# wwood/CoverM

Measured on AMD Instinct MI355X. Metric: aligned reads/s through coverm contig (mean trimmed_mean covered_fraction variance), higher is better.
Workload: dtype i32 depth / u64 sums / f32 estimators

## Files before the change

### coverm_amd/csrc/covermhip.hip

```cpp
#include "pileup_kernels.hip.h"
#include "prep_lean.hip.h"
#include "genome_kernels.hip.h"
#include "sep_kernels.hip.h"
#include "ingest_kernels.hip.h"
#include "group_kernels.hip.h"
#include "sam_kernels.hip.h"
#include "gene_kernels.hip.h"
#include "depth_kernels.hip.h"
#include "depth_bins_kernels.hip.h"
#include "depth_regions_kernels.hip.h"

#include <algorithm>
#include <atomic>
#include <cstddef>
#include <chrono>
#include <cstdio>
#include <dlfcn.h>
#include <functional>
#include <sched.h>
#include <cstdlib>
#include <cstring>
#include <map>
#include <mutex>
#include <string>
// ... 1152 lines not shown
    time_begin(s, COV_K_PREP);
    s->last_gen_all = p.gen_all;
    launch_prep_key((p.want_id ? 4 : 0) | (s->cfg.filter_single ? 2 : 0) | (v.mask != nullptr ? 1 : 0), s, p, v);
    if (v.nT) {
        const u32 n_red = p.gen_all ? 0u : (v.nT + 3u) / 4u, cx_grid0 = (u32)s->n_cus * 8u;
        hipLaunchKernelGGL(k_post_prep, dim3(n_red + cx_grid0), dim3(256), 0, v.st, v.r, s->d_tlen.p, s->d_glob.p, v.cx, v.ti, s->d_ctg.p, v.nT, (const PrepPartial *)s->d_part.p,
                           p.prep_grid, p.prep_chunk, n_red);
    }
    time_end(s, COV_K_PREP);
    HIPCHK(hipGetLastError());
    return COV_OK;
}

static cov_status stage_identity_side(cov_session *s, const PassViews &v) {
    const u32 R = v.R, nT = v.nT;
    if (!s->side) {
        (void)ingest_prep_wait(s);
        if (s->ing.aux && !s->ing.active) s->side = s->ing.aux;
        else { HIPCHK(hipStreamCreateWithFlags(&s->side, hipStreamNonBlocking)); s->side_owned = true; }
    }
    HIPCHK(hipEventRecord(s->ev_prep_done, v.st));
    HIPCHK(hipStreamWaitEvent(s->side, s->ev_prep_done, 0));
    (void)hipEventRecord(s->ev[COV_K_IDENTITY][0], s->side);
    if (s->id_mode) {
        const u32 nch = (R + ID_CH - 1) / ID_CH;
        hipLaunchKernelGGL(k_id_approx, dim3(nch), dim3(256), 0, s->side, v.idp, v.idn, R, s->d_idch.p);
        hipLaunchKernelGGL(k_id_predict, dim3(nT), dim3(64), 0, s->side, s->d_ctg.p, nT, v.idp, v.idn, s->d_idch.p);
        hipLaunchKernelGGL(k_id_exact, dim3(nch), dim3(256), 0, s->side, v.idp, v.idn, R, s->d_idch.p);
        hipLaunchKernelGGL(k_id_combine, dim3(nT), dim3(64), 0, s->side, s->d_ctg.p, nT, v.idp, v.idn, v.r.tid, s->d_idch.p);
    } else
        hipLaunchKernelGGL(k_identity, dim3(nT), dim3(64), 0, s->side, s->d_ctg.p, nT, v.idp, v.idn, v.r.tid);
    (void)hipEventRecord(s->ev[COV_K_IDENTITY][1], s->side);
    s->k_launches[COV_K_IDENTITY]++;
    HIPCHK(hipGetLastError());
    HIPCHK(hipEventRecord(s->ev_side_done, s->side));
    s->ev_fresh = -1;
    return COV_OK;
}

static cov_status stage_ranges(cov_session *s, const FinishPlan &p, const PassViews &v) {
    time_begin(s, COV_K_RANGES);
    const u32 n_blocks = (s->n_tiles + 1023u) / 1024u;
    const u32 cx_grid = (u32)s->n_cus * 8u;
    ScanPair sp{};
    sp.cnt[0] = s->d_tcnt.p; sp.scan[0] = s->d_tscan.p; sp.top[0] = s->d_ttop.p; sp.total[0] = nullptr;
    sp.cnt[1] = s->d_cx_cnt.p; sp.scan[1] = s->d_cx_scan.p; sp.top[1] = s->d_cx_top.p; sp.total[1] = &s->d_glob.p->cx_total;
    hipLaunchKernelGGL(k_tile_scan1, dim3(2u * n_blocks), dim3(1024), 0, v.st, sp, s->n_tiles, n_blocks);
    hipLaunchKernelGGL(k_tile_scan2, dim3(2), dim3(1024), 0, v.st, sp, n_blocks);
    hipLaunchKernelGGL((k_cx_expand<true>), dim3(cx_grid), dim3(256), 0, v.st, v.r, s->d_tlen.p, s->d_glob.p, v.cx, v.ti);
    u32 *slow_list = s->use_fast ? s->d_slow_list.p : nullptr;
    u32 *deep_list = const_cast<u32 *>(pileup_deep_list(s));
    const auto ranges = p.want_hist ? &k_ranges<true> : &k_ranges<false>;
    hipLaunchKernelGGL(ranges, dim3((s->n_tiles + 255) / 256), dim3(256), 0, v.st, s->d_tile_contig.p, s->d_tile_start.p, s->n_tiles, s->d_tlen.p,
                       v.mask, s->d_ctg.p, s->d_desc.p, v.ti, s->d_tscan.p, s->d_ttop.p, v.cx, s->d_glob.p, slow_list, deep_list, s->deep_min);
    time_end(s, COV_K_RANGES);
    HIPCHK(hipGetLastError());
    return COV_OK;
}

static cov_status stage_hist_layout(cov_session *s, const PassViews &v) {
    time_begin(s, COV_K_HIST);
    const u32 hb = (v.nT + 1023u) / 1024u;
    HIPCHK(s->d_hist_top.reserve(hb, v.st));
    hipLaunchKernelGGL((k_hist_sum<0>), dim3(hb), dim3(1024), 0, v.st, (const DevContig *)s->d_ctg.p, v.nT, s->d_tlen.p, v.mask, v.excl, s->d_hist_top.p);
    hipLaunchKernelGGL((k_hist_off<0>), dim3(hb), dim3(1024), 0, v.st, s->d_ctg.p, v.nT, s->d_tlen.p, v.mask, v.excl, (const u64 *)s->d_hist_top.p, s->d_glob.p);
    hipLaunchKernelGGL(k_zero_u32, dim3(2048), dim3(256), 0, v.st, s->d_arena.p, &s->d_glob.p->hist_cap_total);
    time_end(s, COV_K_HIST);
    HIPCHK(hipGetLastError());
    return COV_OK;
}

static cov_status stage_pileup(cov_session *s, const FinishPlan &p, const PassViews &v) {
    const PileupArgs a = pileup_args(s);
    time_begin(s, COV_K_PILEUP);
    if (p.want_hist) launch_any_pileup<true, false>(s, a, s->n_tiles);
    else launch_any_pileup<false, false>(s, a, s->n_tiles);
    if (p.hist_stats_launch) {
        const auto hist_stats = p.est_lanes ? &k_hist_stats<true> : &k_hist_stats<false>;
        hipLaunchKernelGGL(hist_stats, dim3(p.est_lanes ? (v.nT + 255) / 256 : (v.nT + 3) / 4), dim3(256), 0, v.st, s->d_ctg.p, v.nT, (const u32 *)s->d_tlen.p,
                           v.mask, v.excl, (const u32 *)s->d_arena.p);
    }
    time_end(s, COV_K_PILEUP);
    HIPCHK(hipGetLastError());
    return COV_OK;
}

static cov_status stage_hist_compact(cov_session *s, const FinishPlan &p, const PassViews &v) {
    s->hist_prefetched = 0;
    if (p.compacted) {
        HIPCHK(s->d_chist.reserve((size_t)v.R + v.nT + 1, v.st));
        time_begin(s, COV_K_HIST_COMPACT);
        launch_hist_compact(s, v.mask, v.excl);
        time_end(s, COV_K_HIST_COMPACT);
        HIPCHK(hipGetLastError());
        const u64 guess = p.hist_prefetch ? std::min<u64>({s->last_chist_total + s->last_chist_total / 16, (u64)v.R + v.nT + 1, (u64)(64u << 20) / 8}) : 0;
        if (guess) {
            if (guess > s->h_chist_cap) HIPCHK(pinned_grow(s->h_chist, s->h_chist_cap, guess));
            HIPCHK(hipMemcpyAsync(s->h_chist, s->d_chist.p, (size_t)guess * 8, hipMemcpyDeviceToHost, v.st));
            s->hist_prefetched = guess;
        }
    }
    s->hist_fetch_seen = false;
    return COV_OK;
}

static cov_status result_host_bind(cov_session *s, const FinishPlan &p, const PassViews &v) {
    result_host_take(s);
// ... 2110 lines not shown
```

### coverm_amd/csrc/pileup_kernels.hip.h

```cpp
#pragma once
#include <hip/hip_runtime.h>
#include <stdint.h>

#define HSTC_FN __host__ __device__ __forceinline__
#include "hist_stats_core.h"
#define PSCHED_FN __host__ __device__ __forceinline__
#include "pileup_schedule_core.h"
#include "scan_ops.hip.h"

namespace covk {

typedef unsigned long long u64;
typedef unsigned int u32;

constexpr u32 F_POS_UNSORTED = 1u;
constexpr u32 RW_SINGLE = 0u, RW_DOUBLE = 1u, RW_COMPLEX = 2u, RW_BUCKET = 3u;
constexpr u32 FAST_MAX_CAND = 8191u;
constexpr u32 TILE_F_GENERIC = 1u, TILE_F_SLOW = 2u, TILE_F_DEEP = 4u;
constexpr u32 CX_MIN_OPS = 16;

struct DevContig {
    u64 n_primary, n_pass, n_nonsupp, sum_nm, sum_indel;
    double id_primary, id_nonsupp;
    u64 sum_d, sum_d2, cov_win, cov_full, proc_win;
    u64 hist_off;
    u32 first_rec, last_rec;
    u32 rec_start, rec_end;
    u32 n_groups;
    u32 max_span;
    u32 flags;
    u32 hist_cap;
    u32 min_d, max_d;
    u32 hist_len;
    u32 cov_out;
    u64 chist_off;
};
static_assert(sizeof(DevContig) == 160, "DevContig layout");

constexpr u32 COUNTER_SLOTS = 64;
struct DevGlobal {
    u64 first_error;
    u64 hist_cap_total;
    u64 chist_total;
    u32 internal_error;
    u32 n_cx;
    u64 cx_total;
    u32 n_slow;
    u32 n_gen;
    u64 pad2[2];
    u64 prim_slots[COUNTER_SLOTS * 8];
    u64 cons_slots[COUNTER_SLOTS * 8];
    u32 n_deep;
    u32 pad_q[8 * 16 - 1];
};

struct FilterCfg {
    u32 include_improper_pairs, include_supplementary, include_secondary;
    u32 filter_single, min_mapq, min_aligned_length;
    float min_percent_identity, min_aligned_percent;
};

struct Records {
    const int32_t *tid, *pos;
    const uint16_t *flag;
    const uint8_t *mapq;
    const u32 *nm;
    const uint8_t *nm_kind;
    const u32 *l_seq;
    const u32 *cigar_off;
    const u32 *cigar;
    u32 n;
// ... 621 lines not shown
        const u32 L = tlen[tid], t0 = ti.tile_first[tid];
        long long cur0 = r.pos[i];
        u32 wd_next = (u32)lane < nops ? r.cigar[co0 + (u32)lane] : 4u;
        for (u32 base = 0; base < nops; base += 64) {
            const u32 wd = wd_next;
            const u32 idn = base + 64u + (u32)lane;
            wd_next = idn < nops ? r.cigar[co0 + idn] : 4u;
            const u32 len = wd >> 4, bit = 1u << (wd & 15u);
            const u32 fr = (bit & 0x18du) ? len : 0u;
            const u32 incl = (u32)wave_incl_scan((int)fr), excl = incl - fr;
            const long long sj = cur0 + (long long)excl;
            const bool m = (bit & 0x181u) != 0u && len > 0u && sj >= 0 && sj < (long long)L;
            const u32 sv = (u32)sj, ev = sv + len;
            const u32 ts = sv >> ti.shift, te = m ? (min(ev, L) - 1u) >> ti.shift : 0u;
            for (u32 k = 0; __any(m && ts + k <= te); k++) {
                const bool v = m && ts + k <= te;
                const u32 key = t0 + ts + k;
                u32 slot = 0;
                for (u64 todo = __ballot(v); todo != 0;) {
                    const int l = __ffsll((long long)todo) - 1;
                    const u32 k0 = __builtin_amdgcn_readlane(key, l);
                    const u64 grp = __ballot(v && key == k0);
                    u32 b = 0;
                    if (lane == l) b = atomicAdd(FILL ? &cx.cur[k0] : &cx.cnt[k0], (u32)__popcll(grp));
                    if (FILL) {
                        b = __builtin_amdgcn_readlane(b, l);
                        if (v && key == k0) slot = b + (u32)__popcll(grp & lt);
                    }
                    todo &= ~grp;
                }
                if (FILL && v) cx.runs[(u64)cx.cscan[key] + cx.ctop[key >> 10] + slot] = make_uint2(sv, ev);
            }
            cur0 += (long long)__builtin_amdgcn_readlane(incl, 63);
        }
    }
}

template <bool FILL>
__global__ __launch_bounds__(256) void k_cx_expand(Records r, const u32 *__restrict__ tlen, DevGlobal *g, CxIdx cx, TileIdx ti) {
    cx_expand_body<FILL>(r, tlen, g, cx, ti, blockIdx.x * 4u + (threadIdx.x >> 6), gridDim.x * 4u);
}

__global__ __launch_bounds__(256) void k_post_prep(Records r, const u32 *__restrict__ tlen, DevGlobal *g, CxIdx cx, TileIdx ti, DevContig *ctg, u32 n_targets,
                                                   const PrepPartial *__restrict__ part, u32 n_parts, u32 chunk_recs, u32 n_red) {
    if (blockIdx.x < n_red) prep_reduce_body(blockIdx.x * 4u + (threadIdx.x >> 6), ctg, n_targets, part, n_parts, chunk_recs);
    else cx_expand_body<false>(r, tlen, g, cx, ti, (blockIdx.x - n_red) * 4u + (threadIdx.x >> 6), (gridDim.x - n_red) * 4u);
}

template <bool WANT_HIST>
__global__ __launch_bounds__(256) void k_ranges(const u32 *__restrict__ tile_contig, const u32 *__restrict__ tile_start,
                                                u32 n_tiles, const u32 *__restrict__ tlen, const uint8_t *__restrict__ mask,
                                                DevContig *ctg, uint4 *__restrict__ desc, TileIdx ti,
                                                const u32 *__restrict__ tscan, const u32 *__restrict__ ttop, CxIdx cx,
                                                DevGlobal *__restrict__ g, u32 *__restrict__ slow_list, u32 *__restrict__ deep_list, u32 deep_min) {
    const u32 t = blockIdx.x * blockDim.x + threadIdx.x;
    if (t >= n_tiles) return;
    const u32 c = tile_contig[t];
    DevContig *C = &ctg[c];
    uint4 out = make_uint4(0u, 0u, tlen[c], 0u);
    u32 cxn = 0, cxo = 0;
    if (C->n_pass != 0 && (mask == nullptr || mask[c])) {
        const u32 rs = C->rec_start, re = C->rec_end;
        cxn = g->cx_total <= cx.runs_cap ? cx.cnt[t] : 0u;
        cxo = cx.cscan[t] + cx.ctop[t >> 10];
        if (C->n_groups != 1u) out.w = 1u;
        if (C->n_groups != 1u || (C->flags & F_POS_UNSORTED)) {
            out.x = rs; out.y = re;
        } else {
            const u32 tf = ti.tile_first[c];
            const u32 before = (tscan[t] + ttop[t >> 10]) - (tscan[tf] + ttop[tf >> 10]);
            const u32 f = rs + before;
            out.y = min(f + ti.tcnt[t], re);
            out.x = max(min(f, ti.fov[t]), rs);
            out.x = min(out.x, out.y);
        }
    }
    if (out.x < out.y || cxn) {
        if (out.w || out.y - out.x + cxn > FAST_MAX_CAND) {
            out.w |= TILE_F_SLOW;
            if (slow_list != nullptr) slow_list[atomicAdd(&g->n_slow, 1u)] = t;
        }
    }
    if (deep_list != nullptr) {
        const bool deep = (out.x < out.y || cxn) && !(out.w & TILE_F_SLOW) && out.y - out.x + cxn >= deep_min;
        const u64 dm = __ballot(deep);
        if (dm != 0ull) {
            const int lane = lane_id(), lead = __ffsll((long long)dm) - 1;
            u32 base = 0;
            if (lane == lead) base = atomicAdd(&g->n_deep, (u32)__popcll(dm));
            base = (u32)__builtin_amdgcn_readlane((int)base, lead);
            if (deep) {
                out.w |= TILE_F_DEEP;
                deep_list[base + (u32)__popcll(dm & (lane == 0 ? 0ull : (~0ull >> (64 - lane))))] = t;
            }
        }
    }
    if (WANT_HIST) {
        const u32 npass = (u32)min(C->n_pass, (u64)0xffffffffu);
        const u32 cap = min(out.y - out.x + cxn, npass);
        if (__all(c == (u32)__builtin_amdgcn_readfirstlane((int)c))) {
            const u32 m = wave_max_u32(cap);
            if (lane_id() == 0 && m) atomicMax(&C->hist_cap, m);
        } else if (cap) atomicMax(&C->hist_cap, cap);
    }
    desc[2 * t] = out;
    desc[2 * t + 1] = make_uint4(c, tile_start[t], cxo, cxn);
}

template <int MODE>
__device__ __forceinline__ u64 hist_bins_of(const DevContig *C, u32 c, const u32 *__restrict__ tlen, const uint8_t *__restrict__ mask, u64 excl) {
    const bool live = C->n_pass != 0 && (mask == nullptr || mask[c]);
    if (MODE == 0) return live ? (u64)C->hist_cap + 1 : 0;
    return (live && 2 * excl < (u64)tlen[c]) ? (u64)C->max_d + 1 : 0;
}
template <int MODE>
__global__ __launch_bounds__(1024) void k_hist_sum(const DevContig *__restrict__ ctg, u32 n_targets, const u32 *__restrict__ tlen,
                                                   const uint8_t *__restrict__ mask, u64 excl, u64 *__restrict__ top) {
    __shared__ u64 wtot[16];
    const u32 c = blockIdx.x * 1024u + threadIdx.x;
    u64 total;
    (void)block_incl_scan<16>(c < n_targets ? hist_bins_of<MODE>(&ctg[c], c, tlen, mask, excl) : 0ull, wtot, total);
    if (threadIdx.x == 0) top[blockIdx.x] = total;
}
template <int MODE>
__global__ __launch_bounds__(1024) void k_hist_off(DevContig *ctg, u32 n_targets, const u32 *__restrict__ tlen, const uint8_t *__restrict__ mask,
                                                   u64 excl, const u64 *__restrict__ top, DevGlobal *g) {
    __shared__ u64 wtot[16];
    const u64 base = blocks_in_front<16>(top, wtot);
    const u32 c = blockIdx.x * 1024u + threadIdx.x;
    const u64 v = c < n_targets ? hist_bins_of<MODE>(&ctg[c], c, tlen, mask, excl) : 0;
    u64 total;
    const u64 inc = block_incl_scan<16>(v, wtot, total);
    if (c < n_targets) {
        if (MODE == 0) ctg[c].hist_off = base + inc - v;
        else { ctg[c].chist_off = base + inc - v; ctg[c].hist_len = (u32)v; }
    }
    if (blockIdx.x == gridDim.x - 1 && threadIdx.x == 0) {
        if (MODE == 0) g->hist_cap_total = base + total; else g->chist_total = base + total;
    }
}

__global__ void k_zero_u32(u32 *__restrict__ p, const u64 *__restrict__ n_ptr) {
    const u64 n = *n_ptr;
    for (u64 i = (u64)blockIdx.x * blockDim.x + threadIdx.x; i < n; i += (u64)gridDim.x * blockDim.x) p[i] = 0u;
}

__global__ __launch_bounds__(256) void k_hist_compact(const DevContig *__restrict__ ctg, u32 n_targets,
                                                      const u32 *__restrict__ tlen, u64 excl,
                                                      const u32 *__restrict__ arena, u64 *__restrict__ out) {
    const u32 c = blockIdx.x * 4u + (threadIdx.x >> 6);
    if (c >= n_targets) return;
    const DevContig *C = &ctg[c];
    const u32 n = C->hist_len;
    if (n == 0) return;
    const u64 win_len = (u64)tlen[c] - 2 * excl;
    for (u32 d = threadIdx.x & 63u; d < n; d += 64u) {
        u64 v = arena[C->hist_off + d];
        if (d == 0) v += win_len - C->proc_win;
        out[C->chist_off + d] = v;
// ... 521 lines not shown

template <bool WANT_HIST, int HB, int TABLES>
__device__ __forceinline__ void pileup_fast_body(const PileupArgs &a, u32 n_tiles, u32 chunk_tiles, const u32 *__restrict__ deep_list, const u32 *__restrict__ n_deep_ptr) {
    constexpr int TW = FAST_TW, HBW = HB;
    constexpr int DS = TABLES == 1 ? 2 : 0;
    constexpr size_t WB = (size_t)TW * 2 * TABLES + (WANT_HIST ? (size_t)HBW * 4 : 0);
    extern __shared__ __attribute__((aligned(16))) char smem[];
    const int lane = threadIdx.x & 63, w = threadIdx.x >> 6;
    u32 *S = reinterpret_cast<u32 *>(smem + (size_t)w * WB);
    u32 *E = TABLES == 2 ? S + TW / 2 : S;
    u32 *lhist = S + (TW / 2) * TABLES;
    uint4 *S4 = reinterpret_cast<uint4 *>(S), *E4 = reinterpret_cast<uint4 *>(E);
    const u32 wpb = blockDim.x >> 6;
    const u32 wave_id = (u32)__builtin_amdgcn_readfirstlane((int)(blockIdx.x * wpb + (u32)w)), n_waves = gridDim.x * wpb;
    if (WANT_HIST) {
#pragma unroll
        for (int b = lane; b < HBW; b += 64) lhist[b] = 0u;
    }
    u64 sum_d = 0, sum_d2 = 0, proc_win = 0;
    u32 cov_w = 0, cov_f = 0, mn = 0xffffffffu, mx = 0;
    u32 cov_o = 0;
    int cur_c = -1;
    u64 hoff = 0; u32 hcap = 0;
    const u64 excl = a.excl;
    u32 hbound = 0;
    auto drain = [&]() {
        lds_fence();
        for (u32 b = (u32)lane; b <= hbound; b += 64) {
            const u32 x = lhist[b];
            if (x) { atomicAdd(&a.hist_arena[hoff + b], x); lhist[b] = 0u; }
        }
        lds_fence();
        hbound = 0;
    };

    auto hist_add = [&](u32 d, u32 x) {
        if (__builtin_expect(d < (u32)HBW, 1)) atomicAdd(&lhist[d], x);
        else hist_add_overflow(a.hist_arena, hoff, hcap, a.g, d, x);
    };
    auto flush = [&]() {
        if (WANT_HIST) {
            if (cur_c >= 0) {
                drain();
                if (__any(cov_o != 0u)) {
                    const u32 co = wave_sum_u32_dpp(cov_o);
                    if (lane == 0) atomicAdd(&a.ctg[cur_c].cov_out, co);
                }
            }
            cov_o = 0; hbound = 0;
            return;
        }
        if (cur_c >= 0) {
            const bool narrow = !__any((sum_d | sum_d2) >> 50);
            const u64 s1 = narrow ? wave_sum_u56(sum_d) : wave_sum_u64(sum_d), s2 = narrow ? wave_sum_u56(sum_d2) : wave_sum_u64(sum_d2);
            const u32 c1 = wave_sum_u32_dpp(cov_w), c2 = wave_sum_u32_dpp(cov_f);
            const u32 m1 = wave_min_u32_dpp(mn), m2 = wave_max_u32_dpp(mx);
            DevContig *C = &a.ctg[cur_c];
            if (lane == 0) {
                if (s1) atomicAdd(&C->sum_d, s1);
                if (s2) atomicAdd(&C->sum_d2, s2);
                if (c1) atomicAdd(&C->cov_win, (u64)c1);
                if (c2) atomicAdd(&C->cov_full, (u64)c2);
                if (proc_win) {
                    atomicAdd(&C->proc_win, proc_win);
                    atomicMin(&C->min_d, m1);
                    atomicMax(&C->max_d, m2);
                }
            }
        }
        sum_d = sum_d2 = 0; proc_win = 0; cov_w = cov_f = 0; mn = 0xffffffffu; mx = 0;
    };
    auto load_runs = [&](const uint4 &d, uint2 &r0, uint2 &r1) {
        const u32 i0 = d.x + (u32)lane, i1 = i0 + 64u;
        r0 = i0 < d.y ? a.runs[i0] : make_uint2(0u, 0u);
        r1 = i1 < d.y ? a.runs[i1] : make_uint2(0u, 0u);
    };
    const psched::Launch sched = psched::launch_of(n_tiles, chunk_tiles, n_waves, deep_list != nullptr ? *n_deep_ptr : 0u);
    const u32 skip_flags = TILE_F_SLOW | (deep_list != nullptr ? TILE_F_DEEP : 0u);
    psched::Visit vis = psched::first(sched, wave_id);
    if (vis.done) return;
    u32 lt_next = 0;
    u32 t, t_end;
    if (vis.in_list) {
        t = deep_list[vis.idx]; t_end = t + 1u;
        if (vis.idx + n_waves < sched.n_deep) lt_next = deep_list[vis.idx + n_waves];
    } else { t = psched::chunk_t0(sched, vis.idx); t_end = psched::chunk_t1(sched, vis.idx); }
    uint4 ds = a.desc[2 * (size_t)(a.tile_base + t)], dC1 = a.desc[2 * (size_t)(a.tile_base + t) + 1];
    uint2 rw0, rw1;
    load_runs(ds, rw0, rw1);
    for (;;) {
        u32 tn = t + 1, tn_end = t_end;
        psched::Visit visn = vis;
        bool chunk_end = false;
        if (tn >= t_end) {
            chunk_end = true;
            visn = psched::next(sched, wave_id, vis);
            if (visn.done) { tn = 0xffffffffu; tn_end = 0u; }
            else if (visn.in_list) {
                tn = lt_next; tn_end = tn + 1u;
                if (visn.idx + n_waves < sched.n_deep) lt_next = deep_list[visn.idx + n_waves];
            } else { tn = psched::chunk_t0(sched, visn.idx); tn_end = psched::chunk_t1(sched, visn.idx); }
        }
        const bool have_next = tn != 0xffffffffu;
        uint4 nds = make_uint4(0u, 0u, 0u, 0u), ndC1 = make_uint4(0u, 0u, 0u, 0u);
        if (have_next) { nds = a.desc[2 * (size_t)(a.tile_base + tn)]; ndC1 = a.desc[2 * (size_t)(a.tile_base + tn) + 1]; }

        const u32 c = dC1.x, lo = dC1.y, L = ds.z, cxo = dC1.z, cxn = dC1.w;
        const bool live = (ds.x < ds.y || cxn != 0u) && (vis.in_list || !(ds.w & skip_flags));
        uint4 sv0, sv1, ev0, ev1;
        if (live) {
            if ((int)c != cur_c) {
                flush();
                cur_c = (int)c;
                if (WANT_HIST) { hoff = a.ctg[c].hist_off; hcap = a.ctg[c].hist_cap; }
            }
            const u32 zb = TABLES == 2 ? 0u : 0x80008000u;
            const uint4 z4 = make_uint4(zb, zb, zb, zb);
            S4[2 * lane] = z4; S4[2 * lane + 1] = z4;
            if (TABLES == 2) { E4[2 * lane] = z4; E4[2 * lane + 1] = z4; }
            asm volatile("" ::: "memory");
            const u32 hi = lo + TW;
            auto add_run = [&](u32 s, u32 e) {
                if (s < hi && e > lo) {
                    const u32 s0 = s > lo ? s - lo : 0u;
                    atomicAdd(&S[s0 >> 1], (1u << DS) << ((s0 & 1u) << 4));
                    if (e < hi) {
                        const u32 e0 = e - lo;
                        if (TABLES == 2) atomicAdd(&E[e0 >> 1], 1u << ((e0 & 1u) << 4)); else atomicSub(&E[e0 >> 1], (1u << DS) << ((e0 & 1u) << 4));
                    }
                }
            };
            auto apply = [&](const uint2 rw, u32 i) {
                if (rw.y == 0u) return;
                const u32 type = rw.y >> 30;
                if (type <= RW_DOUBLE) {
                    const bool dbl = type == RW_DOUBLE;
                    const u32 l1 = dbl ? (rw.y & 1023u) : rw.y;
                    add_run(rw.x, rw.x + l1);
                    if (dbl) {
                        const u32 s2 = rw.x + l1 + ((rw.y >> 10) & 255u);
                        add_run(s2, s2 + ((rw.y >> 18) & 1023u));
                    }
                } else if (type == RW_COMPLEX) {
                    u32 cursor = (u32)a.r.pos[i];
                    const u32 c0 = a.r.cigar_off[i], c1 = a.r.cigar_off[i + 1];
                    for (u32 k = c0; k < c1; k++) {
                        const u32 wd = a.r.cigar[k];
                        const u32 op = wd & 15u, len = wd >> 4;
                        if (op == 0u || op == 7u || op == 8u) { add_run(cursor, cursor + len); cursor += len; }
                        else if (op == 2u || op == 3u) cursor += len;
                    }
                }
            };
            apply(rw0, ds.x + (u32)lane);
            if (ds.y - ds.x > 64u) {
                apply(rw1, ds.x + 64u + (u32)lane);
                for (u32 i = ds.x + 128u + (u32)lane; i < ds.y; i += 64) apply(a.runs[i], i);
            }
            for (u32 j = (u32)lane; j < cxn; j += 64) { const uint2 q = a.cx_runs[(u64)cxo + j]; add_run(q.x, q.y); }
            asm volatile("" ::: "memory");
            sv0 = S4[2 * lane]; sv1 = S4[2 * lane + 1];
            if (TABLES == 2) { ev0 = E4[2 * lane]; ev1 = E4[2 * lane + 1]; }
        }
        uint2 nrw0 = make_uint2(0u, 0u), nrw1 = make_uint2(0u, 0u);
        if (have_next) load_runs(nds, nrw0, nrw1);

        if (live) {
            const u32 sw[8] = {sv0.x, sv0.y, sv0.z, sv0.w, sv1.x, sv1.y, sv1.z, sv1.w};
            u32 ew[8] = {0u, 0u, 0u, 0u, 0u, 0u, 0u, 0u};
            if (TABLES == 2) { ew[0] = ev0.x; ew[1] = ev0.y; ew[2] = ev0.z; ew[3] = ev0.w; ew[4] = ev1.x; ew[5] = ev1.y; ew[6] = ev1.z; ew[7] = ev1.w; }
            v2i16 dl[8];
#pragma unroll
            for (int k = 0; k < 8; k++) dl[k] = TABLES == 2 ? __builtin_bit_cast(v2i16, sw[k]) - __builtin_bit_cast(v2i16, ew[k]) : __builtin_bit_cast(v2i16, sw[k] ^ 0x80008000u);
            int net = 0;
            const v2i16 one2 = {1, 1};
#pragma unroll
            for (int k = 0; k < 8; k++) net = __builtin_amdgcn_sdot2(dl[k], one2, net, false);
            int d = wave_incl_scan(net) - net;

            const bool has_win = 2 * excl < (u64)L;
            const u32 tlen_t = min((u32)TW, L - lo);
            const u32 ws = has_win ? (u32)excl : 0u, we = has_win ? (u32)(L - excl) : 0u;
            const u32 wst = max(ws, lo), wet = min(we, lo + tlen_t);
            const bool win_any = has_win && wst < wet;
            if (!WANT_HIST && win_any) proc_win += (u64)(wet - wst);
            const bool interior = has_win && lo >= ws && lo + (u32)TW <= we;
            const u32 cand = ds.y - ds.x + cxn;
            const bool fast_tile = interior && cand < (u32)HBW;
            if (WANT_HIST) hbound = max(hbound, min(cand, (u32)HBW - 1u));
            if (WANT_HIST && fast_tile) {
                u32 seg0 = 0;
                u32 da = lds_addr_of(lhist) + ((u32)d << (2 - DS));
#pragma unroll
                for (int j = 0; j < 16; j++) {
                    const int dj = (j & 1) ? (int)dl[j >> 1].y : (int)dl[j >> 1].x;
                    if (j > 0 && dj != 0) { lds_atomic_add(da, (u32)j - seg0); seg0 = (u32)j; }
                    da += (u32)(dj << (2 - DS));
                }
                lds_atomic_add(da, 16u - seg0);
            } else if (WANT_HIST && cand < (u32)HBW) {
                const u32 p0 = lo + 16u * (u32)lane;
                const u32 wa = win_any ? min(max(wst, p0) - p0, 16u) : 0u, wb = win_any ? min(max(wet, p0) - p0, 16u) : 0u;
                const u32 le = min(max(L, p0) - p0, 16u);
                u32 seg0 = 0, covm = 0;
                const u32 da0 = lds_addr_of(lhist);
                u32 da = da0 + ((u32)d << (2 - DS));
#pragma unroll
                for (int j = 0; j < 16; j++) {
                    const int dj = (j & 1) ? (int)dl[j >> 1].y : (int)dl[j >> 1].x;
                    if (j > 0 && dj != 0) {
                        const u32 s_ = max(seg0, wa), e_ = min((u32)j, wb);
                        if (e_ > s_) lds_atomic_add(da, e_ - s_);
                        seg0 = (u32)j;
                    }
                    da += (u32)(dj << (2 - DS));
                    covm = covm + covm + (da != da0 ? 1u : 0u);
                }
                {
                    const u32 s_ = max(seg0, wa);
                    if (wb > s_) lds_atomic_add(da, wb - s_);
                }
                const u32 in_ctg = 0xffffu & ~(0xffffu >> le), in_win = (0xffffu >> wa) & ~(0xffffu >> wb);
                cov_o += (u32)__popc(covm & in_ctg & ~in_win);
            } else if (WANT_HIST) {
                const u32 p0 = lo + 16u * (u32)lane;
                u32 seg0 = 0;
                bool seg_open = false;
#pragma unroll 4
                for (int j = 0; j < 16; j++) {
                    const int dj = (j & 1) ? (int)dl[j >> 1].y : (int)dl[j >> 1].x;
                    const u32 p = p0 + (u32)j;
                    const bool in_w = win_any && p >= wst && p < wet;
                    if (seg_open && (dj != 0 || !in_w)) { hist_add((u32)d >> DS, (u32)j - seg0); seg_open = false; }
                    d += dj;
                    if (in_w) { if (!seg_open) { seg_open = true; seg0 = (u32)j; } }
                    else if (p < L) cov_o += d != 0 ? 1u : 0u;
                }
                if (seg_open) hist_add((u32)d >> DS, 16u - seg0);
            } else if (fast_tile) {
                u32 s1t = 0, s2t = 0, cv = 0;
#pragma unroll
                for (int j = 0; j < 16; j++) {
                    const int dj = (j & 1) ? (int)dl[j >> 1].y : (int)dl[j >> 1].x;
                    d += dj;
                    const u32 du = (u32)d >> DS;
                    s1t += du;
                    s2t = __umul24(du, du) + s2t;
                    cv += du != 0u ? 1u : 0u;
                    mn = min(mn, du); mx = max(mx, du);
                }
                sum_d += s1t; sum_d2 += s2t; cov_w += cv; cov_f += cv;
            } else {
                const u32 p0 = lo + 16u * (u32)lane;
#pragma unroll 4
                for (int j = 0; j < 16; j++) {
                    const int dj = (j & 1) ? (int)dl[j >> 1].y : (int)dl[j >> 1].x;
                    const u32 p = p0 + (u32)j;
                    const bool in_w = win_any && p >= wst && p < wet;
                    d += dj;
                    const u32 du = (u32)d >> DS;
                    if (p < L) cov_f += du != 0u ? 1u : 0u;
                    if (in_w) {
                        sum_d += du; sum_d2 += (u64)du * du;
                        cov_w += du != 0u ? 1u : 0u;
                        mn = min(mn, du); mx = max(mx, du);
                    }
                }
            }
        }
        if (chunk_end) { flush(); cur_c = -1; }
        if (!have_next) break;
        t = tn; t_end = tn_end; vis = visn; ds = nds; dC1 = ndC1; rw0 = nrw0; rw1 = nrw1;
    }
}

template <bool WANT_HIST>
__global__ __launch_bounds__(256) __attribute__((amdgpu_waves_per_eu(8, 8))) void k_pileup_fast(PileupArgs a, u32 n_tiles, u32 chunk_tiles, const u32 *__restrict__ deep_list, const u32 *__restrict__ n_deep) {
    pileup_fast_body<WANT_HIST, FAST_HB, 1>(a, n_tiles, chunk_tiles, deep_list, n_deep);
}
template <bool WANT_HIST>
__global__ __launch_bounds__(256) __attribute__((amdgpu_waves_per_eu(6, 6))) void k_pileup_fast2t(PileupArgs a, u32 n_tiles, u32 chunk_tiles, const u32 *__restrict__ deep_list, const u32 *__restrict__ n_deep) {
    pileup_fast_body<WANT_HIST, FAST_HB7, 2>(a, n_tiles, chunk_tiles, deep_list, n_deep);
}


struct DevEstimator { int kind; float min_frac; u64 excl; int exclude_mismatches; float trim_min, trim_max; u32 pad; };
static_assert(sizeof(DevEstimator) == 32, "DevEstimator mirrors cov_estimator");
constexpr u32 EST_MAX = 16;
struct EstParams { DevEstimator e[EST_MAX]; u32 n; u32 pad; };
enum { EST_MEAN = 0, EST_TRIMMED_MEAN = 1, EST_PILEUP_COUNTS = 2, EST_COVERED_FRACTION = 3, EST_COVERED_BASES = 4, EST_RPKM = 5, EST_TPM = 6,
       EST_VARIANCE = 7, EST_LENGTH = 8, EST_READ_COUNT = 9, EST_READS_PER_BASE = 10, EST_ANIR = 11 };

__device__ __forceinline__ float est_f32(u64 x) { return __ull2float_rn(x); }
__device__ __forceinline__ u64 est_f32_to_usize(float x) {
    if (!(x == x) || x <= 0.0f) return 0ull;
    if (x >= 18446744073709551616.0f) return ~0ull;
    return (u64)x;
}

template <typename BIN>
__device__ __forceinline__ u64 trimmed_total_wave(const BIN *__restrict__ bins, u32 nh, u64 bin0_extra, u64 min_index, u64 max_index) {
    const int lane = lane_id();
    u64 total = 0, carry = 0;
    int state = 0;
    for (u32 b = 0; b < nh && state < 2; b += 64) {
        const u32 i = b + (u32)lane;
        u64 n = i < nh ? (u64)bins[i] : 0ull;
        if (i == 0) n += bin0_extra;
        const u64 acc = carry + wave_incl_scan_u64(n);
        const bool valid = i < nh;
        int first = 0;
        if (state == 0) {
            const u64 sm = __ballot(valid && acc >= min_index);
            if (sm == 0) { carry = bcast_u64(acc, 63); continue; }
            const int ls = __ffsll((long long)sm) - 1;
            const u64 acc_s = bcast_u64(acc, ls);
            total = (acc_s > max_index ? max_index - min_index + 1 : acc_s - min_index + 1) * (u64)(b + (u32)ls);
            state = 1; first = ls + 1;
        }
        const u64 em = __ballot(valid && lane >= first && acc > max_index);
        const int le = em ? __ffsll((long long)em) - 1 : 64;
        u64 part = (valid && lane >= first && lane < le) ? n * (u64)i : 0ull;
        if (em && lane == le) {
            const u64 excess = acc - n;
            part = (max_index >= excess ? max_index - excess + 1 : 0ull) * (u64)i;
// ... 267 lines not shown
```

### coverm_amd/csrc/scan_ops.hip.h

```cpp
#pragma once
#include <hip/hip_runtime.h>
#include <stdint.h>

namespace covsc {

typedef unsigned long long u64;
typedef unsigned int u32;

struct Plus { template <typename T> __device__ __forceinline__ T operator()(T a, T b) const { return a + b; } };
struct Max { template <typename T> __device__ __forceinline__ T operator()(T a, T b) const { return a < b ? b : a; } };

__device__ __forceinline__ int lane_id() { return threadIdx.x & 63; }

__device__ __forceinline__ int wave_incl_scan(int v) {
    v += __builtin_amdgcn_update_dpp(0, v, 0x111, 0xf, 0xf, false);
    v += __builtin_amdgcn_update_dpp(0, v, 0x112, 0xf, 0xf, false);
    v += __builtin_amdgcn_update_dpp(0, v, 0x114, 0xf, 0xf, false);
    v += __builtin_amdgcn_update_dpp(0, v, 0x118, 0xf, 0xf, false);
    v += __builtin_amdgcn_update_dpp(0, v, 0x142, 0xa, 0xf, false);
    v += __builtin_amdgcn_update_dpp(0, v, 0x143, 0xc, 0xf, false);
    return v;
}
__device__ __forceinline__ u32 wave_incl_scan(u32 v) { return (u32)wave_incl_scan((int)v); }
__device__ __forceinline__ int wave_incl_max(int v) {
    const int NEG = (int)0x80000000;
    v = max(v, __builtin_amdgcn_update_dpp(NEG, v, 0x111, 0xf, 0xf, false));
    v = max(v, __builtin_amdgcn_update_dpp(NEG, v, 0x112, 0xf, 0xf, false));
    v = max(v, __builtin_amdgcn_update_dpp(NEG, v, 0x114, 0xf, 0xf, false));
    v = max(v, __builtin_amdgcn_update_dpp(NEG, v, 0x118, 0xf, 0xf, false));
    v = max(v, __builtin_amdgcn_update_dpp(NEG, v, 0x142, 0xa, 0xf, false));
    v = max(v, __builtin_amdgcn_update_dpp(NEG, v, 0x143, 0xc, 0xf, false));
    return v;
}
template <typename T, typename Op>
__device__ __forceinline__ T wave_incl_scan(T v, Op op) {
    const int lane = lane_id();
#pragma unroll
    for (int o = 1; o < 64; o <<= 1) { const T t = __shfl_up(v, o); if (lane >= o) v = op(v, t); }
    return v;
}
__device__ __forceinline__ u32 wave_incl_scan(u32 v, Plus) { return wave_incl_scan(v); }
__device__ __forceinline__ u64 wave_incl_scan_u64(u64 v) { return wave_incl_scan(v, Plus{}); }

__device__ __forceinline__ u64 wave_sum_u64(u64 v) {
#pragma unroll
    for (int o = 32; o > 0; o >>= 1) v += __shfl_xor(v, o);
    return v;
}
__device__ __forceinline__ u32 wave_sum_u32(u32 v) {
#pragma unroll
    for (int o = 32; o > 0; o >>= 1) v += __shfl_xor(v, o);
    return v;
}
__device__ __forceinline__ u32 wave_min_u32(u32 v) {
#pragma unroll
    for (int o = 32; o > 0; o >>= 1) v = min(v, (u32)__shfl_xor(v, o));
    return v;
}
__device__ __forceinline__ u32 wave_max_u32(u32 v) {
#pragma unroll
    for (int o = 32; o > 0; o >>= 1) v = max(v, (u32)__shfl_xor(v, o));
    return v;
}

__device__ __forceinline__ u32 wave_sum_u32_dpp(u32 v) { return (u32)__builtin_amdgcn_readlane(wave_incl_scan((int)v), 63); }
__device__ __forceinline__ u64 wave_sum_u56(u64 v) {
    const u32 lo = (u32)v & 0xffffffu, hi = (u32)(v >> 24);
    return (u64)wave_sum_u32_dpp(lo) + ((u64)wave_sum_u32_dpp(hi) << 24);
}
__device__ __forceinline__ u32 wave_max_u32_dpp(u32 v) {
    return (u32)__builtin_amdgcn_readlane(wave_incl_max((int)(v ^ 0x80000000u)), 63) ^ 0x80000000u;
}
__device__ __forceinline__ u32 wave_min_u32_dpp(u32 v) { return ~wave_max_u32_dpp(~v); }


template <int NW, typename T, typename Op = Plus>
__device__ __forceinline__ T block_incl_scan(T v, T *lds, T &total, Op op = Op{}) {
    const int lane = lane_id(), w = (int)(threadIdx.x >> 6);
    const T inc = wave_incl_scan(v, op);
    if (lane == 63) lds[w] = inc;
    __syncthreads();
    T wbase = T(0), tot = T(0);
#pragma unroll
    for (int k = 0; k < NW; k++) { const T x = lds[k]; if (k < w) wbase = op(wbase, x); tot = op(tot, x); }
    __syncthreads();
    total = tot;
    return op(wbase, inc);
}
template <int NW, typename T>
__device__ __forceinline__ T block_prev(T x, T *lds, T first) {
    const int lane = lane_id(), w = (int)(threadIdx.x >> 6);
    const T up = __shfl_up(x, 1);
    if (lane == 63) lds[w] = x;
    __syncthreads();
    const T prev = lane ? up : (w ? lds[w - 1] : first);
    __syncthreads();
    return prev;
}
template <int NW, typename S, typename T, typename Op = Plus>
__device__ __forceinline__ T blocks_in_front(const S *__restrict__ top, T *lds, Op op = Op{}) {
    T mine = T(0), base;
    for (u32 b = threadIdx.x; b < blockIdx.x; b += NW * 64u) mine = op(mine, (T)top[b]);
    (void)block_incl_scan<NW>(mine, lds, base, op);
    return base;
}

constexpr u32 SCAN_ITEMS = 16, SCAN_BLOCK = 256 * SCAN_ITEMS;

template <typename F>
__global__ __launch_bounds__(256) void k_scan_sums(F f, u32 n, u32 *__restrict__ block_sums) {
    __shared__ u32 wsum[4];
    const u32 i0 = blockIdx.x * SCAN_BLOCK + threadIdx.x * SCAN_ITEMS;
    u32 s = 0;
    for (u32 k = 0; k < SCAN_ITEMS; k++) if (i0 + k < n) s += f(i0 + k);
    u32 total;
    (void)block_incl_scan<4>(s, wsum, total);
    if (threadIdx.x == 0) block_sums[blockIdx.x] = total;
}
__global__ __launch_bounds__(1024) void k_scan_offsets(u32 *__restrict__ block_sums, u32 nb, u64 *__restrict__ total64) {
    __shared__ u64 part[1024];
    const u32 t = threadIdx.x, per = (nb + 1023u) / 1024u, k0 = t * per, k1 = min(nb, k0 + per);
// ... 23 lines not shown
```

Before: 50.72 billion.

## Precompute tile liveness and window class bits in range kernel

```diff
diff --git a/coverm_amd/csrc/covermhip.hip b/coverm_amd/csrc/covermhip.hip
--- a/coverm_amd/csrc/covermhip.hip
+++ b/coverm_amd/csrc/covermhip.hip
@@ -1228,7 +1228,7 @@
     u32 *deep_list = const_cast<u32 *>(pileup_deep_list(s));
     const auto ranges = p.want_hist ? &k_ranges<true> : &k_ranges<false>;
     hipLaunchKernelGGL(ranges, dim3((s->n_tiles + 255) / 256), dim3(256), 0, v.st, s->d_tile_contig.p, s->d_tile_start.p, s->n_tiles, s->d_tlen.p,
-                       v.mask, s->d_ctg.p, s->d_desc.p, v.ti, s->d_tscan.p, s->d_ttop.p, v.cx, s->d_glob.p, slow_list, deep_list, s->deep_min);
+                       v.mask, s->d_ctg.p, s->d_desc.p, v.ti, s->d_tscan.p, s->d_ttop.p, v.cx, s->d_glob.p, slow_list, deep_list, s->deep_min, v.excl);
     time_end(s, COV_K_RANGES);
     HIPCHK(hipGetLastError());
     return COV_OK;
diff --git a/coverm_amd/csrc/pileup_kernels.hip.h b/coverm_amd/csrc/pileup_kernels.hip.h
--- a/coverm_amd/csrc/pileup_kernels.hip.h
+++ b/coverm_amd/csrc/pileup_kernels.hip.h
@@ -6,6 +6,8 @@
 #include "hist_stats_core.h"
 #define PSCHED_FN __host__ __device__ __forceinline__
 #include "pileup_schedule_core.h"
+#define PTILE_FN __host__ __device__ __forceinline__
+#include "pileup_tile_class_core.h"
 #include "scan_ops.hip.h"
 
 namespace covk {
@@ -17,6 +19,7 @@
 constexpr u32 RW_SINGLE = 0u, RW_DOUBLE = 1u, RW_COMPLEX = 2u, RW_BUCKET = 3u;
 constexpr u32 FAST_MAX_CAND = 8191u;
 constexpr u32 TILE_F_GENERIC = 1u, TILE_F_SLOW = 2u, TILE_F_DEEP = 4u;
+static_assert(((TILE_F_GENERIC | TILE_F_SLOW | TILE_F_DEEP) & (ptile::F_LIVE | ptile::F_INTERIOR | ptile::F_NOWIN)) == 0u, "tile descriptor flags overlap");
 constexpr u32 CX_MIN_OPS = 16;
 
 struct DevContig {
@@ -744,7 +747,7 @@
                                                 u32 n_tiles, const u32 *__restrict__ tlen, const uint8_t *__restrict__ mask,
                                                 DevContig *ctg, uint4 *__restrict__ desc, TileIdx ti,
                                                 const u32 *__restrict__ tscan, const u32 *__restrict__ ttop, CxIdx cx,
-                                                DevGlobal *__restrict__ g, u32 *__restrict__ slow_list, u32 *__restrict__ deep_list, u32 deep_min) {
+                                                DevGlobal *__restrict__ g, u32 *__restrict__ slow_list, u32 *__restrict__ deep_list, u32 deep_min, u64 excl) {
     const u32 t = blockIdx.x * blockDim.x + threadIdx.x;
     if (t >= n_tiles) return;
     const u32 c = tile_contig[t];
@@ -795,8 +798,10 @@
             if (lane_id() == 0 && m) atomicMax(&C->hist_cap, m);
         } else if (cap) atomicMax(&C->hist_cap, cap);
     }
+    const u32 lo = tile_start[t];
+    out.w |= ptile::class_bits(out.z, lo, excl, out.x, out.y, cxn);
     desc[2 * t] = out;
-    desc[2 * t + 1] = make_uint4(c, tile_start[t], cxo, cxn);
+    desc[2 * t + 1] = make_uint4(c, lo, cxo, cxn);
 }
 
 template <int MODE>
@@ -1424,7 +1429,7 @@
         }
         if (cur_c >= 0) {
             const bool narrow = !__any((sum_d | sum_d2) >> 50);
-            const u64 s1 = narrow ? wave_sum_u56(sum_d) : wave_sum_u64(sum_d), s2 = narrow ? wave_sum_u56(sum_d2) : wave_sum_u64(sum_d2);
+            const u64 s1 = narrow ? wave_sum_u56(sum_d) : wave_sum_u64_dpp(sum_d), s2 = narrow ? wave_sum_u56(sum_d2) : wave_sum_u64_dpp(sum_d2);
             const u32 c1 = wave_sum_u32_dpp(cov_w), c2 = wave_sum_u32_dpp(cov_f);
             const u32 m1 = wave_min_u32_dpp(mn), m2 = wave_max_u32_dpp(mx);
             DevContig *C = &a.ctg[cur_c];
@@ -1448,37 +1453,34 @@
         r1 = i1 < d.y ? a.runs[i1] : make_uint2(0u, 0u);
     };
     const psched::Launch sched = psched::launch_of(n_tiles, chunk_tiles, n_waves, deep_list != nullptr ? *n_deep_ptr : 0u);
-    const u32 skip_flags = TILE_F_SLOW | (deep_list != nullptr ? TILE_F_DEEP : 0u);
+    const u32 live_mask_chunk = ptile::F_LIVE | TILE_F_SLOW | (deep_list != nullptr ? TILE_F_DEEP : 0u), live_mask_list = ptile::F_LIVE;
     psched::Visit vis = psched::first(sched, wave_id);
     if (vis.done) return;
     u32 lt_next = 0;
-    u32 t, t_end;
+    u32 t, t_end, live_mask;
     if (vis.in_list) {
-        t = deep_list[vis.idx]; t_end = t + 1u;
+        t = deep_list[vis.idx]; t_end = t + 1u; live_mask = live_mask_list;
         if (vis.idx + n_waves < sched.n_deep) lt_next = deep_list[vis.idx + n_waves];
-    } else { t = psched::chunk_t0(sched, vis.idx); t_end = psched::chunk_t1(sched, vis.idx); }
+    } else { t = psched::chunk_t0(sched, vis.idx); t_end = psched::chunk_t1(sched, vis.idx); live_mask = live_mask_chunk; }
     uint4 ds = a.desc[2 * (size_t)(a.tile_base + t)], dC1 = a.desc[2 * (size_t)(a.tile_base + t) + 1];
     uint2 rw0, rw1;
     load_runs(ds, rw0, rw1);
     for (;;) {
-        u32 tn = t + 1, tn_end = t_end;
-        psched::Visit visn = vis;
-        bool chunk_end = false;
-        if (tn >= t_end) {
-            chunk_end = true;
-            visn = psched::next(sched, wave_id, vis);
-            if (visn.done) { tn = 0xffffffffu; tn_end = 0u; }
-            else if (visn.in_list) {
-                tn = lt_next; tn_end = tn + 1u;
-                if (visn.idx + n_waves < sched.n_deep) lt_next = deep_list[visn.idx + n_waves];
-            } else { tn = psched::chunk_t0(sched, visn.idx); tn_end = psched::chunk_t1(sched, visn.idx); }
-        }
-        const bool have_next = tn != 0xffffffffu;
-        uint4 nds = make_uint4(0u, 0u, 0u, 0u), ndC1 = make_uint4(0u, 0u, 0u, 0u);
-        if (have_next) { nds = a.desc[2 * (size_t)(a.tile_base + tn)]; ndC1 = a.desc[2 * (size_t)(a.tile_base + tn) + 1]; }
-
         const u32 c = dC1.x, lo = dC1.y, L = ds.z, cxo = dC1.z, cxn = dC1.w;
-        const bool live = (ds.x < ds.y || cxn != 0u) && (vis.in_list || !(ds.w & skip_flags));
+        const bool live = (ds.w & live_mask) == ptile::F_LIVE;
+        u32 tn = t + 1u;
+        const bool visit_end = tn == t_end;
+        bool last = false;
+        if (visit_end) {
+            vis = psched::next(sched, wave_id, vis);
+            if (vis.done) { tn = t; last = true; }
+            else if (vis.in_list) {
+                tn = lt_next; t_end = tn + 1u;
+                if (vis.idx + n_waves < sched.n_deep) lt_next = deep_list[vis.idx + n_waves];
+            } else { tn = psched::chunk_t0(sched, vis.idx); t_end = psched::chunk_t1(sched, vis.idx); live_mask = live_mask_chunk; }
+        }
+        const uint4 nds = a.desc[2 * (size_t)(a.tile_base + tn)], ndC1 = a.desc[2 * (size_t)(a.tile_base + tn) + 1];
+
         uint4 sv0, sv1, ev0, ev1;
         if (live) {
             if ((int)c != cur_c) {
@@ -1534,8 +1536,8 @@
             sv0 = S4[2 * lane]; sv1 = S4[2 * lane + 1];
             if (TABLES == 2) { ev0 = E4[2 * lane]; ev1 = E4[2 * lane + 1]; }
         }
-        uint2 nrw0 = make_uint2(0u, 0u), nrw1 = make_uint2(0u, 0u);
-        if (have_next) load_runs(nds, nrw0, nrw1);
+        uint2 nrw0, nrw1;
+        load_runs(nds, nrw0, nrw1);
 
         if (live) {
             const u32 sw[8] = {sv0.x, sv0.y, sv0.z, sv0.w, sv1.x, sv1.y, sv1.z, sv1.w};
@@ -1550,13 +1552,7 @@
             for (int k = 0; k < 8; k++) net = __builtin_amdgcn_sdot2(dl[k], one2, net, false);
             int d = wave_incl_scan(net) - net;
 
-            const bool has_win = 2 * excl < (u64)L;
-            const u32 tlen_t = min((u32)TW, L - lo);
-            const u32 ws = has_win ? (u32)excl : 0u, we = has_win ? (u32)(L - excl) : 0u;
-            const u32 wst = max(ws, lo), wet = min(we, lo + tlen_t);
-            const bool win_any = has_win && wst < wet;
-            if (!WANT_HIST && win_any) proc_win += (u64)(wet - wst);
-            const bool interior = has_win && lo >= ws && lo + (u32)TW <= we;
+            const bool interior = (ds.w & ptile::F_INTERIOR) != 0u;
             const u32 cand = ds.y - ds.x + cxn;
             const bool fast_tile = interior && cand < (u32)HBW;
             if (WANT_HIST) hbound = max(hbound, min(cand, (u32)HBW - 1u));
@@ -1572,7 +1568,8 @@
                 lds_atomic_add(da, 16u - seg0);
             } else if (WANT_HIST && cand < (u32)HBW) {
                 const u32 p0 = lo + 16u * (u32)lane;
-                const u32 wa = win_any ? min(max(wst, p0) - p0, 16u) : 0u, wb = win_any ? min(max(wet, p0) - p0, 16u) : 0u;
+                const ptile::Window win = ptile::tile_window_of(ds.w, L, lo, excl);
+                const u32 wa = min(max(win.wst, p0) - p0, 16u), wb = min(max(win.wet, p0) - p0, 16u);
                 const u32 le = min(max(L, p0) - p0, 16u);
                 u32 seg0 = 0, covm = 0;
                 const u32 da0 = lds_addr_of(lhist);
@@ -1596,13 +1593,14 @@
                 cov_o += (u32)__popc(covm & in_ctg & ~in_win);
             } else if (WANT_HIST) {
                 const u32 p0 = lo + 16u * (u32)lane;
+                const ptile::Window win = ptile::tile_window_of(ds.w, L, lo, excl);
                 u32 seg0 = 0;
                 bool seg_open = false;
 #pragma unroll 4
                 for (int j = 0; j < 16; j++) {
                     const int dj = (j & 1) ? (int)dl[j >> 1].y : (int)dl[j >> 1].x;
                     const u32 p = p0 + (u32)j;
-                    const bool in_w = win_any && p >= wst && p < wet;
+                    const bool in_w = p >= win.wst && p < win.wet;
                     if (seg_open && (dj != 0 || !in_w)) { hist_add((u32)d >> DS, (u32)j - seg0); seg_open = false; }
                     d += dj;
                     if (in_w) { if (!seg_open) { seg_open = true; seg0 = (u32)j; } }
@@ -1611,6 +1609,7 @@
                 if (seg_open) hist_add((u32)d >> DS, 16u - seg0);
             } else if (fast_tile) {
                 u32 s1t = 0, s2t = 0, cv = 0;
+                proc_win += (u64)TW;
 #pragma unroll
                 for (int j = 0; j < 16; j++) {
                     const int dj = (j & 1) ? (int)dl[j >> 1].y : (int)dl[j >> 1].x;
@@ -1624,11 +1623,13 @@
                 sum_d += s1t; sum_d2 += s2t; cov_w += cv; cov_f += cv;
             } else {
                 const u32 p0 = lo + 16u * (u32)lane;
+                const ptile::Window win = ptile::tile_window_of(ds.w, L, lo, excl);
+                proc_win += (u64)(win.wet - win.wst);
 #pragma unroll 4
                 for (int j = 0; j < 16; j++) {
                     const int dj = (j & 1) ? (int)dl[j >> 1].y : (int)dl[j >> 1].x;
                     const u32 p = p0 + (u32)j;
-                    const bool in_w = win_any && p >= wst && p < wet;
+                    const bool in_w = p >= win.wst && p < win.wet;
                     d += dj;
                     const u32 du = (u32)d >> DS;
                     if (p < L) cov_f += du != 0u ? 1u : 0u;
@@ -1640,9 +1641,11 @@
                 }
             }
         }
-        if (chunk_end) { flush(); cur_c = -1; }
-        if (!have_next) break;
-        t = tn; t_end = tn_end; vis = visn; ds = nds; dC1 = ndC1; rw0 = nrw0; rw1 = nrw1;
+        if (visit_end) {
+            flush(); cur_c = -1;
+            if (last) break;
+        }
+        t = tn; ds = nds; dC1 = ndC1; rw0 = nrw0; rw1 = nrw1;
     }
 }
 
diff --git a/coverm_amd/csrc/pileup_tile_class_core.h b/coverm_amd/csrc/pileup_tile_class_core.h
--- /dev/null
+++ b/coverm_amd/csrc/pileup_tile_class_core.h
@@ -0,0 +1,43 @@
+#pragma once
+#include <stdint.h>
+
+#ifndef PTILE_FN
+#define PTILE_FN inline
+#endif
+
+namespace ptile {
+
+typedef unsigned int u32;
+typedef unsigned long long u64;
+
+constexpr u32 TILE_W = 1024u;
+constexpr u32 F_LIVE = 8u;
+constexpr u32 F_INTERIOR = 16u;
+constexpr u32 F_NOWIN = 32u;
+
+PTILE_FN bool has_window(u32 L, u64 excl) { return 2ull * excl < (u64)L; }
+
+struct Window { u32 wst, wet; };
+PTILE_FN Window tile_window(u32 L, u32 lo, u64 excl) {
+    const bool hw = has_window(L, excl);
+    const u32 ws = hw ? (u32)excl : 0u, we = hw ? (u32)((u64)L - excl) : 0u;
+    const u32 rest = L - lo, tlen = rest < TILE_W ? rest : TILE_W, te = lo + tlen;
+    return Window{ws > lo ? ws : lo, we < te ? we : te};
+}
+
+PTILE_FN u32 class_bits(u32 L, u32 lo, u64 excl, u32 x, u32 y, u32 cxn) {
+    u32 f = 0u;
+    if (x < y || cxn != 0u) f |= F_LIVE;
+    const bool hw = has_window(L, excl);
+    if (hw && (u64)lo >= excl && (u64)lo + TILE_W <= (u64)L - excl) f |= F_INTERIOR;
+    const Window w = tile_window(L, lo, excl);
+    if (!hw || !(w.wst < w.wet)) f |= F_NOWIN;
+    return f;
+}
+
+PTILE_FN Window tile_window_of(u32 flags, u32 L, u32 lo, u64 excl) {
+    if (flags & F_NOWIN) return Window{0u, 0u};
+    return tile_window(L, lo, excl);
+}
+
+}
diff --git a/coverm_amd/csrc/scan_ops.hip.h b/coverm_amd/csrc/scan_ops.hip.h
--- a/coverm_amd/csrc/scan_ops.hip.h
+++ b/coverm_amd/csrc/scan_ops.hip.h
@@ -67,6 +67,10 @@
 __device__ __forceinline__ u64 wave_sum_u56(u64 v) {
     const u32 lo = (u32)v & 0xffffffu, hi = (u32)(v >> 24);
     return (u64)wave_sum_u32_dpp(lo) + ((u64)wave_sum_u32_dpp(hi) << 24);
+}
+__device__ __forceinline__ u64 wave_sum_u64_dpp(u64 v) {
+    const u32 p0 = (u32)v & 0xffffffu, p1 = (u32)(v >> 24) & 0xffffffu, p2 = (u32)(v >> 48);
+    return (u64)wave_sum_u32_dpp(p0) + ((u64)wave_sum_u32_dpp(p1) << 24) + ((u64)wave_sum_u32_dpp(p2) << 48);
 }
 __device__ __forceinline__ u32 wave_max_u32_dpp(u32 v) {
     return (u32)__builtin_amdgcn_readlane(wave_incl_max((int)(v ^ 0x80000000u)), 63) ^ 0x80000000u;
```

New measurement: 50.34 billion (median of 2 runs). No clear change (-0.8%).
